# Hiroshiba/realtime-yukarin

Hardware: AMD Instinct MI355X
Metric: acoustic frames/s (stage1+stage2 fwd) @16kHz/5ms (higher is better)
Workload: dtype f32; 1 GPU; BASELINE config #3: stage-1 + stage-2 SR forward, buffer_time 0.5 s + 2x0.5 s convert_extra_time @16 kHz / 5 ms -> 300 real frames (384 padded) per window, 1 window(s) per GPU per step, SYN-64 random-init weights; model=SYN-64, frames=300, padded_frames=384, windows_per_gpu=1, lanes_per_gpu=2

## Files before the change

### realtime_yukarin_amd/csrc/ry_exec.cpp

```cpp
#include "ry_kernels.h"
#include "ry_plan.h"

static void fill_geom(RyConvGeom& g, const Layer& l, const LayerPlan& lp, int B, const float* s1, int C1, const float* s2, int C2) {
    memset(&g, 0, sizeof g);
    const TapTable t = make_taps(l);
    g.src1 = s1; g.src2 = s2; g.C1 = C1; g.C2 = C2; g.S1 = C1; g.S2 = C2;
    if (lp.path == PATH_IGEMM_BF16 && lp.x3) { g.C1 = 3 * C1; g.C2 = 3 * C2; g.S1 = 2 * C1; g.S2 = 2 * C2; }
    g.B = B; g.Hi = lp.Hi; g.Wi = lp.Wi; g.Ho = lp.Ho; g.Wo = lp.Wo;
    g.Hs = lp.Hi; g.Hos = lp.Ho;
    if (lp.crop_hi > 0) { g.Hi = lp.crop_hi; g.Ho = l.deconv ? 2 * lp.crop_hi : lp.crop_hi; }
    if (l.deconv) { g.Mh = g.Hi; g.Mw = lp.Wi; g.stride = 1; g.pad = 0; g.ostride = 2; }
    else { g.Mh = g.Ho; g.Mw = lp.Wo; g.stride = l.stride; g.pad = l.pad; g.ostride = 1; }
    g.nphases = t.nphases; g.ntaps = t.ntaps; g.N = l.cout; g.kw = l.deconv ? 2 : l.k; g.dil = l.deconv ? 1 : l.dil;
    const size_t esize = lp.path == PATH_IGEMM_BF16 ? 2 : 4;
    g.zoff1 = (unsigned)((size_t)B * lp.Hi * lp.Wi * g.S1 * esize); g.zoff2 = (unsigned)((size_t)B * lp.Hi * lp.Wi * g.S2 * esize);
    if (lp.crop_hi > 0 && lp.crop_lo > 0) {
        const size_t o1 = (size_t)lp.crop_lo * lp.Wi * g.S1 * esize, o2 = (size_t)lp.crop_lo * lp.Wi * g.S2 * esize;
        g.src1 = reinterpret_cast<const float*>(reinterpret_cast<const char*>(s1) + o1); g.zoff1 -= (unsigned)o1;
        if (s2) { g.src2 = reinterpret_cast<const float*>(reinterpret_cast<const char*>(s2) + o2); g.zoff2 -= (unsigned)o2; }
    }
    for (int ph = 0; ph < 4; ++ph) {
        g.pdy[ph] = (signed char)t.pdy[ph]; g.pdx[ph] = (signed char)t.pdx[ph];
        for (int tt = 0; tt < 16; ++tt) { g.tdy[ph][tt] = (signed char)t.dy[ph][tt]; g.tdx[ph][tt] = (signed char)t.dx[ph][tt]; }
    }
// ... 190 lines not shown
        while ((1 << p.tw_shift) < tw) ++p.tw_shift;
        p.th = th;
    }
    dim3 grid((unsigned)(((p.s.mtiles * p.s.ntiles * g.nphases * lp.splits + 7) / 8) * 8));
    RY_TRY(Lc.begin(tile_name(lp.tile, lp.kg, bf16, patch), l.name, lp.flops, lp.bytes, grid));
#define RY_IGEMM_LAUNCH(BM_, BN_, WM_, WN_, BF16_)                                                                                        \
    do {                                                                                                                                 \
        if (patch == 1 && lp.kg == 2) RY_LAUNCH((ry_igemm_ldsdma<BM_, BN_, WM_, WN_, 2, BF16_, 1>), grid, 512, Lc.stream, p);            \
        else if (patch == 1) RY_LAUNCH((ry_igemm_ldsdma<BM_, BN_, WM_, WN_, 1, BF16_, 1>), grid, 256, Lc.stream, p);                     \
        else if (patch == 2 && lp.kg == 2) RY_LAUNCH((ry_igemm_ldsdma<BM_, BN_, WM_, WN_, 2, BF16_, 2>), grid, 512, Lc.stream, p);       \
        else if (patch == 2) RY_LAUNCH((ry_igemm_ldsdma<BM_, BN_, WM_, WN_, 1, BF16_, 2>), grid, 256, Lc.stream, p);                     \
        else if (lp.kg == 2) RY_LAUNCH((ry_igemm_ldsdma<BM_, BN_, WM_, WN_, 2, BF16_, 0>), grid, 512, Lc.stream, p);                     \
        else RY_LAUNCH((ry_igemm_ldsdma<BM_, BN_, WM_, WN_, 1, BF16_, 0>), grid, 256, Lc.stream, p);                                     \
    } while (0)
#define RY_IGEMM_TILES(BF16_)                                                   \
    switch (lp.tile) {                                                          \
        case TILE_128x128: RY_IGEMM_LAUNCH(128, 128, 2, 2, BF16_); break;       \
        case TILE_96x128: RY_IGEMM_LAUNCH(96, 128, 1, 4, BF16_); break;         \
        case TILE_64x128: RY_IGEMM_LAUNCH(64, 128, 1, 4, BF16_); break;         \
        case TILE_128x64: RY_IGEMM_LAUNCH(128, 64, 4, 1, BF16_); break;         \
        default: RY_IGEMM_LAUNCH(32, 128, 1, 4, BF16_); break;                  \
    }
    if (bf16) RY_IGEMM_TILES(true) else RY_IGEMM_TILES(false)
#undef RY_IGEMM_TILES
#undef RY_IGEMM_LAUNCH
    RY_TRY(Lc.end());
    return launch_tail(Lc, l, lp, B, g.Ho, slope);
}

static int launch_conv2d(Launcher& Lc, const Layer& l, const LayerPlan& lp, int B, const float* s1, int C1, const float* s2, int C2, float slope) {
    if (lp.path == PATH_OS2D) return launch_c2d_os(Lc, l, lp, B, s1, C1, s2, C2, slope);
    if (lp.path == PATH_WINO) return launch_wino(Lc, l, lp, B, s1, C1, s2, C2, slope);
    if (lp.path == PATH_IGEMM || lp.path == PATH_IGEMM_BF16) return launch_igemm(Lc, l, lp, B, s1, C1, s2, C2, slope);
    if (lp.path == PATH_FIRST) {
        RySrFirstParams p;
        p.x = s1; p.w = l.wdir; p.scale = l.scale; p.shift = l.shift; p.out16 = lp.w16 ? lp.out16 : nullptr;
        p.out = (lp.w32 || !p.out16) ? lp.out : nullptr;
        p.x3 = lp.o16x3 ? 1 : 0;
        p.B = B; p.H = lp.Hi; p.W = lp.Wi; p.N = l.cout; p.act = l.act; p.slope = slope;
        const int quads = l.cout / 4;
        p.qshift = -1;
        for (int sh = 0; sh < 16; ++sh) if ((1 << sh) == quads) p.qshift = sh;
        const long long per_row = (long long)((lp.Wi + 3) / 4) * quads;
        dim3 grid((unsigned)((per_row + 255) / 256), (unsigned)lp.Hi, (unsigned)B);
        if (grid.y > 65535u || grid.z > 65535u) return fail(RY_EINVAL, "%s: %u rows x %u windows exceed the grid limit", l.name, grid.y, grid.z);
        RY_TRY(Lc.begin("ry_sr_first", l.name, lp.flops, lp.bytes, grid));
        RY_LAUNCH((ry_sr_first<4>), grid, 256, Lc.stream, p);
        RY_TRY(Lc.end());
    } else if (lp.path == PATH_LAST) {
        RySrLastParams p;
        p.src1 = s1; p.src2 = s2; p.C1 = C1; p.C2 = C2; p.w = l.wdir; p.scale = l.scale; p.shift = l.shift;
        p.out = lp.out; p.B = B; p.H = lp.Hi; p.W = lp.Wi;
        p.rows_valid = lp.last_rows; p.out_cols = lp.last_cols; p.do_exp = lp.last_exp;
        p.row0 = lp.last_row0; p.out_rows = lp.last_out_rows > 0 ? lp.last_out_rows : lp.last_rows;
        const long long total = (long long)B * p.rows_valid * lp.Wi;
        dim3 grid((unsigned)((total + 7) / 8));
        if (C1 + C2 == 128 && lp.Wi % 16 == 0) {
            const long long strips = (long long)B * p.rows_valid * (lp.Wi / 16);
            p.xcd_band = 1;
            const long long nb = (strips + 7) / 8;
            dim3 sg((unsigned)(((nb + 7) / 8) * 8));
            RY_TRY(Lc.begin("ry_sr_last<false>", l.name, lp.flops, lp.bytes, sg));
            RY_LAUNCH(ry_sr_last<false>, sg, 256, Lc.stream, p);
        } else {
            RY_TRY(Lc.begin("ry_sr_last_gather", l.name, lp.flops, lp.bytes, grid));
            RY_LAUNCH(ry_sr_last_gather, grid, 256, Lc.stream, p);
        }
// ... 76 lines not shown
            break;
        default:
            RY_OS_CASE_NU(RY_C1D_DECONV) RY_OS_CASE(RY_C1D_DECONV, 4, 4) RY_OS_CASE(RY_C1D_DECONV, 2, 8) RY_OS_CASE(RY_C1D_DECONV, 2, 4)
            return fail(RY_EINVAL, "%s: no ry_c1d_os instantiation for slice %dx%d", l.name, lp.os_cb, lp.os_tp);
            break;
    }
#undef RY_OS_CASE
#undef RY_OS_CASE_NU
#undef RY_OS_CASE_PM
    return Lc.end();
}

static RySrc1d src1d_of(const ry_net* net, const Plan& P, int idx) {
    RySrc1d s;
    memset(&s, 0, sizeof s);
    if (idx == -2) { s.C = 0; s.Craw = 1; s.splits = 1; return s; }
    if (idx == -1) {
        s.raw = P.mode == 1 ? P.x_in : P.cur_in; s.C = net->desc.in_ch; s.Craw = s.C; s.splits = 1; s.act = RY_ACT_NONE;
        return s;
    }
    const Layer& l = net->layers[idx];
    const LayerPlan& lp = P.lp[idx];
    s.raw = lp.raw; s.scale = l.scale; s.shift = l.shift; s.slab_stride = lp.slab_stride;
    s.C = l.act == RY_ACT_GLU ? l.cout / 2 : l.cout; s.Craw = l.cout; s.splits = lp.splits; s.act = l.act;
    return s;
}

static int enqueue_forward(ry_net* net, Plan& P, Launcher& Lc) {
    const ry_net_desc& d = net->desc;
    const int lo = 0, hi = 16;
    const int nd = d.ndim, B = P.B;
    const float slope = d.lrelu_slope;
    const bool padfuse_now = plan_padfuse_now(net, P);
    if (P.mode == 1 && !padfuse_now) {
        const int cols_in = nd == 1 ? d.in_ch : d.width + 1;
        const int cols_out = nd == 1 ? d.in_ch : d.width;
        RyPadRowsParams q;
        q.in = P.cur_in; q.minv = nullptr; q.out = P.x_in;
        q.rows_in = P.n_frames; q.cols_in = cols_in; q.rows_out = P.T; q.cols_out = cols_out; q.take_log = nd == 2;
        q.in_bstride = (long long)P.n_frames * cols_in; q.out_bstride = (long long)P.T * cols_out; q.minv_bstride = cols_in;
        dim3 pg((unsigned)((cols_in + 15) / 16), (unsigned)B);
        RY_TRY(Lc.begin("ry_pad_min_rows", "pad", 0, 4.0 * B * (P.n_frames * cols_in + P.T * cols_out), pg));
        if (P.n_frames > 128) RY_LAUNCH(ry_pad_min_rows<64>, pg, 1024, Lc.stream, q);
        else RY_LAUNCH(ry_pad_min_rows<16>, pg, 256, Lc.stream, q);
        RY_TRY(Lc.end());
    }
    const WindowRows rows = plan_window_rows(net, P);
    for (int i = lo; i < hi; ++i) {
        const Layer& l = net->layers[i];
        const LayerPlan& lp = P.lp[i];
        if (nd == 1 && P.s1_os) {
            const bool fused_pad = l.src_a < 0 && padfuse_now;
            const float* sa = l.src_a < 0 ? ((P.mode == 1 && !padfuse_now) ? P.x_in : P.cur_in) : P.lp[l.src_a].out;
            const float* sb = l.src_b < 0 ? nullptr : P.lp[l.src_b].out;
            const int keep = (i == 15 && P.mode == 1) ? P.n_frames : lp.Wo;
            RY_TRY(launch_c1d_os(Lc, l, lp, B, sa, l.cin_a, sb, l.cin_b, i == 15 ? P.cur_out : lp.out, keep, slope, fused_pad ? P.n_frames : 0));
        } else if (nd == 1) {
            RY_TRY(launch_conv1d(Lc, l, lp, B, src1d_of(net, P, l.src_a), src1d_of(net, P, l.src_b), slope));
        } else {
            const bool in16 = lp.path == PATH_IGEMM_BF16;
            const float* s1 = l.src_a < 0 ? (P.mode == 1 ? P.x_in : P.cur_in)
                                          : in16 ? reinterpret_cast<const float*>(P.lp[l.src_a].out16) : P.lp[l.src_a].out;
            const float* s2 = l.src_b < 0 ? nullptr : in16 ? reinterpret_cast<const float*>(P.lp[l.src_b].out16) : P.lp[l.src_b].out;
            LayerPlan lq = lp;
            if (i == 15 && (P.mode == 0 || lp.path == PATH_LAST)) lq.out = P.cur_out;
            if (i == 15 && P.mode == 1 && lp.path == PATH_LAST) {
                lq.last_rows = rows.k1 - rows.k0; lq.last_row0 = rows.k0; lq.last_out_rows = P.n_frames; lq.flops = lp.flops * (rows.k1 - rows.k0) / lp.Ho;
            }
            if (rows.hole_n[i] > 0) { lq.hole_lo = rows.hole_lo[i]; lq.hole_n = rows.hole_n[i]; lq.flops = lp.flops * (lp.Ho - rows.hole_n[i]) / lp.Ho; }
            if (rows.crop_hi[i] > 0) {
                lq.crop_hi = rows.crop_hi[i]; lq.crop_lo = rows.crop_lo[i]; lq.flops = lp.flops * rows.crop_hi[i] / lp.Hi; lq.bytes = lp.bytes * rows.crop_hi[i] / lp.Hi;
            }
            RY_TRY(launch_conv2d(Lc, l, lq, B, s1, l.cin_a, s2, l.cin_b, slope));
        }
    }
    if (nd == 1 && P.s1_os) {
    } else if (nd == 1) {
        RyMaterializeParams m;
        m.s = src1d_of(net, P, 15); m.L = P.T; m.keep = P.mode == 1 ? P.n_frames : P.T;
        m.npix = (long long)B * m.keep; m.slope = slope;
        m.out = P.cur_out;
        dim3 mg((unsigned)((m.npix * d.out_ch + 255) / 256));
        RY_TRY(Lc.begin("ry_materialize", "decoder/c7", 0, 4.0 * m.npix * d.out_ch * 2, mg));
        RY_LAUNCH(ry_materialize, mg, 256, Lc.stream, m);
        RY_TRY(Lc.end());
    } else if (P.mode == 1 && P.lp[15].path != PATH_LAST) {
        RySrPostParams q;
        q.y = P.lp[15].out; q.out = P.cur_out; q.rows = P.n_frames; q.cols_in = d.width; q.cols_out = d.width + 1;
        q.y_bstride = (long long)P.T * d.width; q.out_bstride = (long long)P.n_frames * (d.width + 1);
        dim3 pg((unsigned)(((long long)P.n_frames * (d.width + 1) + 255) / 256), (unsigned)B);
        RY_TRY(Lc.begin("ry_sr_post", "post", 0, 8.0 * B * P.n_frames * (d.width + 1), pg));
        RY_LAUNCH(ry_sr_post, pg, 256, Lc.stream, q);
        RY_TRY(Lc.end());
    }
    return RY_OK;
}

int autotune_plan(ry_net* net, Plan& P) {
    ry_ctx* ctx = net->ctx;
    const int B = P.B;
    const float slope = net->desc.lrelu_slope;
// ... 436 lines not shown
```

### realtime_yukarin_amd/csrc/ry_host.h

```cpp
#pragma once
#include "ry_dev.h"

#include "../../include/ry355.h"

#include <cmath>
#include <cstdarg>
#include <cstdio>
#include <cstdlib>
#include <chrono>
#include <cstring>
#include <map>
#include <memory>
#include <string>
#include <tuple>
#include <vector>

namespace rt {
#ifdef RY_HOST_EMU
typedef int err_t;
static const char* err_str(err_t) { return "emu"; }
static err_t set_device(int) { return 0; }
static err_t device_count(int* n) { *n = 1; return 0; }
static err_t stream_create(ry_stream_t* s) { *s = nullptr; return 0; }
static err_t stream_destroy(ry_stream_t) { return 0; }
// ... 125 lines not shown
    float* wigx3 = nullptr;
    int cin() const { return cin_a + cin_b; }
};

enum { PATH_IGEMM = 1, PATH_DIRECT = 2, PATH_FIRST = 3, PATH_LAST = 4, PATH_IGEMM_BF16 = 5,
       PATH_IGEMM_X3 = 6,
       PATH_OS2D = 7,
       PATH_WINO = 8 };
enum { TILE_128x128 = 1, TILE_64x128 = 3, TILE_32x128 = 4, TILE_128x64 = 5, TILE_96x128 = 6 };

struct LayerPlan {
    int Hi = 1, Wi = 1, Ho = 1, Wo = 1;
    int splits = 1;
    long long slab_stride = 0;
    float* raw = nullptr;
    int os_cb = 0, os_tp = 0, os_kt = 0;
    int path = 0, tile = 0;
    bool any_m_patch = false;
    int os2_mt4 = 0, os2_nt4 = 0, os2_waves = 0, os2_depth = 0;
    int wino_cfg = 0, wino_mbw = 0;
    const float* wwin = nullptr;
    int kg = 1;
    float* out = nullptr;
    unsigned short* out16 = nullptr;
    bool w32 = true, w16 = false;
    bool x3 = false;
    bool o16x3 = false;
    float* slabs = nullptr;
    int hole_lo = 0, hole_n = 0;
    int crop_hi = 0;
    int crop_lo = 0;
    int last_rows = 0, last_cols = 0, last_exp = 0;
    int last_row0 = 0, last_out_rows = 0;
    double flops = 0, bytes = 0;
    double flops_exec = 0;
};

inline void keep_rows(int n_frames, int disc_front, int disc_back, int* k0, int* k1) {
    *k0 = disc_front < n_frames ? disc_front : 0;
    *k1 = n_frames - disc_back > *k0 ? n_frames - disc_back : n_frames;
}

struct Plan {
    int B = 0, T = 0;
    int mode = 0;
    int n_frames = 0;
    int disc_front = 0, disc_back = 0;
    Arena arena;
    std::vector<LayerPlan> lp;
    float* user_in = nullptr;
    float* user_out = nullptr;
    float* x_in = nullptr;
    size_t user_in_floats = 0, user_out_floats = 0;
    bool s1_os = false;
    bool s1_padfuse = false;
    const float* cur_in = nullptr;
    float* cur_out = nullptr;
#ifndef RY_HOST_EMU
    struct GraphSlot { const float* in; float* out; hipGraphExec_t gexec; bool tried; long long graph_n, last_n; unsigned long long used; };
    std::vector<GraphSlot> gslots;
    unsigned long long gclock = 0;
    ~Plan() { for (GraphSlot& g : gslots) if (g.gexec) hipGraphExecDestroy(g.gexec); }
#endif
};

struct KernelRec {
    std::string name, layer;
    double flops, bytes, flops_exec;
    int grid[3];
};

struct ry_net {
    int dtype = 0;
    ry_ctx* ctx = nullptr;
    ry_stream_t stream = nullptr;
    rt::Event done;
    bool has_done = false;
    ry_net_desc desc;
    std::vector<Layer> layers;
    std::shared_ptr<Arena> weights = std::make_shared<Arena>();
    std::map<std::tuple<int, int, int, int>, std::unique_ptr<Plan>> plans;
    Plan* last_plan = nullptr;
    bool use_graph = true;
    std::vector<KernelRec>* rec = nullptr;
    std::vector<std::pair<rt::Event, rt::Event>>* rec_events = nullptr;
};

static int upload(Arena& a, ry_ctx* ctx, const std::vector<float>& h, float** d) {
// ... 35 lines not shown
```

### realtime_yukarin_amd/csrc/ry_kernels.h

```cpp
#pragma once
#include "ry_dev.h"


RY_DEV float ry_act(float v, int act, float slope) {
    if (act == RY_ACT_LRELU) return v >= 0.f ? v : v * slope;
    if (act == RY_ACT_RELU) return v > 0.f ? v : 0.f;
    return v;
}
RY_DEV float ry_sigmoid(float v) { return 1.f / (1.f + expf(-v)); }

RY_DEV int ry_fdiv(int x, int d, float inv_d) {
    int q = (int)((float)x * inv_d);
    const int r = x - q * d;
    q += (r >= d) ? 1 : 0;
    q -= (r < 0) ? 1 : 0;
    return q;
}

RY_DEV void ry_keep2(float& a, float& b) {
#ifndef RY_HOST_EMU
    asm volatile("" : "+v"(a), "+v"(b));
#endif
}
RY_DEV int ry_bitrev(int v, int bits) {
// ... 1068 lines not shown
    const int Ctot = g.C1 + g.C2;
    float acc = 0.f;
    for (int t = 0; t < g.ntaps; ++t) {
        const int iy = yb + g.tdy[phase][t], ix = xb + g.tdx[phase][t];
        if ((unsigned)iy >= (unsigned)g.Hi || (unsigned)ix >= (unsigned)g.Wi) continue;
        const size_t pix = (size_t)(b * g.Hs + iy) * g.Wi + ix;
        const float* w = p.wd + ((size_t)(phase * g.ntaps + t) * Ctot) * g.N + n;
        const float* s1 = g.src1 + pix * g.C1;
        for (int c = 0; c < g.C1; ++c) acc = fmaf(s1[c], w[(size_t)c * g.N], acc);
        if (g.C2 > 0) {
            const float* s2 = g.src2 + pix * g.C2;
            const float* w2 = w + (size_t)g.C1 * g.N;
            for (int c = 0; c < g.C2; ++c) acc = fmaf(s2[c], w2[(size_t)c * g.N], acc);
        }
    }
    const size_t ob = (size_t)(b * g.Hos + ry * g.ostride + g.pdy[phase]) * g.Wo + rx * g.ostride + g.pdx[phase];
    p.out[ob * g.N + n] = ry_act(fmaf(acc, p.scale[n], p.shift[n]), p.act, p.slope);
}

struct RySrFirstParams {
    const float* x;
    const float* w;
    const float* scale;
    const float* shift;
    float* out;
    unsigned short* out16;
    int x3;
    int B, H, W, N;
    int act;
    float slope;
    int qshift;
};

template <int PX>
RY_KERNEL(256) void ry_sr_first(RySrFirstParams p) {
    const int quads = p.N >> 2;
    const int gpr = (p.W + PX - 1) / PX;
    const int idx = (int)blockIdx.x * 256 + (int)threadIdx.x;
    const int gx = p.qshift >= 0 ? idx >> p.qshift : idx / quads;
    const int cq = idx - gx * quads;
    if (gx >= gpr) return;
    const int y = (int)blockIdx.y, b = (int)blockIdx.z;
    const int x0 = gx * PX;
    f32x4 wr[9];
#pragma unroll
    for (int t = 0; t < 9; ++t) wr[t] = ry_ld4(p.w + (size_t)t * p.N + cq * 4);
    const f32x4 sc = ry_ld4(p.scale + cq * 4), sh = ry_ld4(p.shift + cq * 4);
    float xv[3][PX + 2];
#pragma unroll
    for (int dy = 0; dy < 3; ++dy) {
        const int iy = y + dy - 1;
#pragma unroll
        for (int j = 0; j < PX + 2; ++j) {
            const int ix = x0 + j - 1;
            xv[dy][j] = ((unsigned)iy < (unsigned)p.H && (unsigned)ix < (unsigned)p.W) ? p.x[((size_t)b * p.H + iy) * p.W + ix] : 0.f;
        }
    }
#pragma unroll
    for (int j = 0; j < PX; ++j) {
        if (x0 + j >= p.W) break;
        f32x4 acc = {0.f, 0.f, 0.f, 0.f};
#pragma unroll
        for (int t = 0; t < 9; ++t) {
            const float xs_ = xv[t / 3][j + t % 3];
#pragma unroll
            for (int u = 0; u < 4; ++u) acc[u] = fmaf(xs_, wr[t][u], acc[u]);
        }
        f32x4 o;
#pragma unroll
        for (int u = 0; u < 4; ++u) o[u] = ry_act(fmaf(acc[u], sc[u], sh[u]), p.act, p.slope);
        const size_t oi = (((size_t)b * p.H + y) * p.W + x0 + j) * p.N + cq * 4;
        if (p.out) ry_st4(p.out + oi, o);
        if (p.out16) {
            if (p.x3) ry_st4_bf16_x3(p.out16, ((size_t)b * p.H + y) * p.W + x0 + j, p.N, cq * 4, o);
            else ry_st4_bf16(p.out16 + oi, o);
        }
    }
}

struct RySrLastParams {
    const float* src1;
    const float* src2;
    int C1, C2;
    const float* w;
    const float* scale;
    const float* shift;
    float* out;
    int B, H, W;
    int rows_valid;
    int row0;
    int out_rows;
    int out_cols;
    int do_exp;
    int xcd_band;
};

RY_KERNEL(256) void ry_sr_last_gather(RySrLastParams p) {
    const int l = (int)threadIdx.x & 31;
    const long long pix = (long long)blockIdx.x * 8 + (threadIdx.x >> 5);
    const long long total = (long long)p.B * p.rows_valid * p.W;
    const bool live = pix < total;
    const long long pp = live ? pix : 0;
    const int x = (int)(pp % p.W);
    const int y = (int)((pp / p.W) % p.rows_valid) + p.row0;
    const int b = (int)(pp / ((long long)p.W * p.rows_valid));
    const int Ctot = p.C1 + p.C2;
    float acc = 0.f;
    if (live) {
        for (int t = 0; t < 9; ++t) {
// ... 630 lines not shown
```

### realtime_yukarin_amd/csrc/ry_plan.cpp

```cpp
#include "ry_plan.h"

static const int ENC_CH[8] = {1, 2, 4, 8, 8, 8, 8, 8};
static const int DEC_IN[7] = {8, 16, 16, 16, 16, 8, 4};
static const int DEC_OUT[7] = {8, 8, 8, 8, 4, 2, 1};

std::vector<Layer> build_topology(const ry_net_desc& d) {
    std::vector<Layer> L(16);
    const int B = d.base, e = d.extensive_layers;
    const int end_k = e > 0 ? 3 : 1;
    const int g = (d.glu && d.ndim == 1) ? 2 : 1;
    const int blk_act_e = g == 2 ? RY_ACT_GLU : RY_ACT_LRELU, blk_act_d = g == 2 ? RY_ACT_GLU : RY_ACT_RELU;
    auto nm = [](Layer& l, const char* p, int i) { snprintf(l.name, sizeof l.name, "%s/c%d", p, i); };
    {
        Layer& l = L[0]; nm(l, "encoder", 0);
        l.k = end_k; l.stride = 1; l.pad = end_k / 2; l.cin_a = d.in_ch; l.cout = B; l.src_a = -1; l.act = RY_ACT_LRELU;
    }
    for (int i = 1; i < 8; ++i) {
        Layer& l = L[i]; nm(l, "encoder", i);
        const bool down = i < e;
        l.k = down ? 4 : 1; l.stride = down ? 2 : 1; l.pad = down ? 1 : 0;
        l.cin_a = ENC_CH[i - 1] * B; l.cout = ENC_CH[i] * B * g; l.src_a = i - 1; l.bn = true; l.act = blk_act_e;
    }
    for (int j = 0; j < 7; ++j) {
        Layer& l = L[8 + j]; nm(l, "decoder", j);
// ... 228 lines not shown
        relayout_direct(l, W, w);
        RY_TRY(upload(arena, ctx, w, &l.wdir));
    }
    return RY_OK;
}

static int g_poison = 0;
int poison_fill(ry_ctx* ctx, float* p, size_t nfloats) {
    if (!g_poison || !p || !nfloats) return RY_OK;
    RT_TRY(rt::dmemset(p, 0xFF, nfloats * sizeof(float), ctx->stream));
    RT_TRY(rt::stream_sync(ctx->stream));
    return RY_OK;
}
int alloc_ztail(ry_ctx* ctx, Arena& arena, float** p, size_t nfloats) {
    RY_TRY(arena.alloc(p, nfloats + ZTAIL));
    if (g_poison) RT_TRY(rt::dmemset(*p, 0xFF, nfloats * sizeof(float), ctx->stream));
    RT_TRY(rt::dmemset(*p + nfloats, 0, ZTAIL * sizeof(float), ctx->stream));
    RT_TRY(rt::stream_sync(ctx->stream));
    return RY_OK;
}

void tile_dims(int tile, int* bm, int* bn) {
    switch (tile) {
        case TILE_128x128: *bm = 128; *bn = 128; break;
        case TILE_64x128: *bm = 64; *bn = 128; break;
        case TILE_128x64: *bm = 128; *bn = 64; break;
        case TILE_96x128: *bm = 96; *bn = 128; break;
        default: *bm = 32; *bn = 128; break;
    }
}


static int g_s2_hole = 1;
static int g_s2_crop = 2;
static LayerForce g_force[16];
bool layer_plan_fixed(int i) { return g_force[i].fixed(); }
int g_x3_min_m = 128;
int g_autotune = 0;
int g_autotune_reps = 3, g_autotune_max = 0;
int g_autotune_pick = -1;
const char* tile_name(int tile, int kg, bool bf16, int patch) {
    {
        static std::map<int, std::string> names;
        const int key = ((tile * 4 + kg) * 2 + (bf16 ? 1 : 0)) * 4 + patch;
        auto it = names.find(key);
        if (it == names.end()) {
            int bm, bn; tile_dims(tile, &bm, &bn);
            const int wmv = (tile == TILE_128x128) ? 2 : (tile == TILE_128x64 ? 4 : 1), wnv = 4 / wmv;
            char buf[96];
            snprintf(buf, sizeof buf, "ry_igemm_ldsdma<%d,%d,%d,%d,%d,%s,%d>", bm, bn, wmv, wnv, kg == 2 ? 2 : 1, bf16 ? "true" : "false", patch);
            it = names.emplace(key, buf).first;
        }
        return it->second.c_str();
    }
}

static thread_local double g_plan_peak = 157.3e6;
static thread_local int g_plan_ck = 32;
static const double g_x3_peak = 2.0e9, g_x3_kg2 = 1.15;
static thread_local double g_plan_kg2 = 1.0;

int tile_occ(int tile, int kg) {
    int bm, bn; tile_dims(tile, &bm, &bn);
    const int occ = (160 * 1024) / (kg * (bm + bn) * 32 * 4 * 2 + bm * 16);
    const int cap = 4 / kg;
    return occ > cap ? cap : occ;
// ... 224 lines not shown

static int ensure_wwin(ry_net* net, int i, const float** out) {
    auto& lazy = net->weights->lazy;
    auto it = lazy.find(i);
    if (it == lazy.end()) {
        float* d = nullptr;
        RY_TRY(upload_wwin(net->ctx, *net->weights, net->layers[i], &d));
        it = lazy.emplace(i, d).first;
    }
    *out = it->second;
    return RY_OK;
}

bool plan_tile_rows(const LayerPlan& lp, int Mh, int Mw, int* th, int* tw_out) {
    if (lp.path == PATH_WINO) {
        int tw; wino_tile_hw(lp.wino_cfg, lp.wino_mbw, th, &tw);
        if (tw_out) *tw_out = tw;
        return Mh % *th == 0 && Mw % tw == 0;
    }
    int bm, bn; tile_dims(lp.tile, &bm, &bn);
    for (int tw = 16; tw >= 4; tw >>= 1)
        if (bm % tw == 0 && Mw % tw == 0 && Mh % (bm / tw) == 0) { *th = bm / tw; if (tw_out) *tw_out = tw; return true; }
    return false;
}

bool plan_hole_ok(const Layer& l, const LayerPlan& lp, int lo, int n) {
    const bool igemm = lp.path == PATH_IGEMM || lp.path == PATH_IGEMM_BF16;
    if ((!igemm && lp.path != PATH_WINO) || (igemm && lp.splits != 1) || l.deconv || lp.crop_hi > 0 || (lp.Wo * l.cout) % 8) return false;
    int th = 1, tw = 0;
    if (!plan_tile_rows(lp, lp.Ho, lp.Wo, &th, &tw) || (igemm && tw != 16)) return false;
    return n > 0 && lo >= 1 && lo % th == 0 && n % th == 0 && lo + n <= lp.Ho;
}

WindowRows plan_window_rows(const ry_net* net, const Plan& P) {
    const int nd = net->desc.ndim, B = P.B;
    WindowRows w;
    w.k1 = P.n_frames;
    if (nd == 2 && P.mode == 1 && P.lp[15].path == PATH_LAST) {
        keep_rows(P.n_frames, P.disc_front, P.disc_back, &w.k0, &w.k1);
    }
    if (nd == 2 && P.mode == 1 && g_s2_crop && P.lp[15].path == PATH_LAST && net->layers[15].src_a == 14) {
        int need0 = w.k0 > 0 ? w.k0 - 1 : 0, need1 = w.k1 + 1;
        for (int i = 14; i >= 8; --i) {
            const Layer& l = net->layers[i];
            const LayerPlan& lp = P.lp[i];
            if (need1 > lp.Ho) need1 = lp.Ho;
            if (need0 <= 0 && need1 >= lp.Ho) break;
            if (lp.path != PATH_IGEMM && lp.path != PATH_IGEMM_BF16 && lp.path != PATH_WINO) break;
            if (l.src_a != i - 1) break;
            int r0, r1;
            if (l.deconv) { r0 = need0 > 0 ? (need0 - 1) / 2 : 0; r1 = need1 / 2 + 1; }
            else if (l.k == 1 && l.stride == 1) { r0 = need0; r1 = need1; }
            else break;
            const int Mw = l.deconv ? lp.Wi : lp.Wo, Mh = l.deconv ? lp.Hi : lp.Ho;
            int th = 1;
            if (plan_tile_rows(lp, Mh, Mw, &th)) { r0 = r0 / th * th; r1 = (r1 + th - 1) / th * th; }
            if (r1 > lp.Hi) r1 = lp.Hi;
            if (r0 <= 0 && r1 >= lp.Hi) break;
            int bm = 256, bn = 64;
            if (lp.path == PATH_WINO) { if (lp.wino_cfg == 2) bm = 512; } else tile_dims(lp.tile, &bm, &bn);
            const long wgs = (long)(((long)B * Mh * Mw + bm - 1) / bm) * (l.cout / bn) * (l.deconv ? 4 : 1) * lp.splits;
            if (g_s2_crop >= 2 || wgs > 256) { w.crop_lo[i] = r0; w.crop_hi[i] = r1 - r0; need0 = r0; need1 = r1; }
            else { need0 = 0; need1 = lp.Hi; }
        }
    }
    if (nd == 2 && P.mode == 1 && g_s2_hole && P.n_frames < P.T - 2) {
// ... 111 lines not shown
    }
    if (nd == 1) {
        P.s1_os = true;
        for (int i = 0; i < 16; ++i) if (!c1d_os_capable(net->layers[i]) || !net->layers[i].w1os) P.s1_os = false;
        P.s1_padfuse = P.s1_os && P.mode == 1 && c1d_mode(net->layers[0]) == RY_C1D_S1 && net->layers[0].cin() <= 64;
    }
    for (int i = 0; i < 16; ++i) {
        const Layer& l = net->layers[i];
        LayerPlan& lp = P.lp[i];
        const size_t out_elems = (size_t)B * lp.Ho * lp.Wo * l.cout;
        if (nd == 1 && P.s1_os) {
            plan_s1_os(l, lp, B);
            if (i < 15) {
                RY_TRY(P.arena.alloc(&lp.out, out_elems));
                RY_TRY(poison_fill(net->ctx, lp.out, out_elems));
            }
        } else if (nd == 1) {
            const int mode = c1d_mode(l);
            lp.splits = choose_splits_1d(l, B, mode == RY_C1D_DECONV ? lp.Wi : lp.Wo, mode);
            lp.slab_stride = (long long)out_elems;
            RY_TRY(P.arena.alloc(&lp.raw, out_elems * lp.splits));
            RY_TRY(poison_fill(net->ctx, lp.raw, out_elems * lp.splits));
        } else {
            RY_TRY(alloc_ztail(net->ctx, P.arena, &lp.out, out_elems));
            bool src16 = l.src_a >= 0;
            for (int src : {l.src_a, l.src_b}) {
                const int sp = src >= 0 ? P.lp[src].path : 0;
                if (src >= 0 && sp != PATH_FIRST && sp != PATH_IGEMM && sp != PATH_IGEMM_BF16 && sp != PATH_OS2D) src16 = false;
            }
            RY_TRY(plan_s2_layer(net->ctx, P.arena, l, lp, B, net->dtype, g_force[i], src16, i == 15, P.mode));
            if (lp.path == PATH_WINO) RY_TRY(ensure_wwin(net, i, &lp.wwin));
        }
    }
    if (nd == 2 && net->dtype != 0) {
        const bool x3 = net->dtype == 2;
        std::vector<char> need32(16, 0), need16(16, 0);
        need32[15] = 1;
        for (int i = 0; i < 16; ++i)
            for (int src : {net->layers[i].src_a, net->layers[i].src_b})
                if (src >= 0) (P.lp[i].path == PATH_IGEMM_BF16 ? need16 : need32)[src] = 1;
        for (int i = 0; i < 16; ++i) {
            LayerPlan& lp = P.lp[i];
            lp.w32 = need32[i] || lp.path == PATH_DIRECT || lp.path == PATH_LAST; lp.w16 = need16[i];
            lp.o16x3 = x3;
            if (lp.w16) {
                float* q = nullptr;
                RY_TRY(alloc_ztail(net->ctx, P.arena, &q, ((size_t)B * lp.Ho * lp.Wo * net->layers[i].cout * (x3 ? 2 : 1) + 1) / 2));
                lp.out16 = reinterpret_cast<unsigned short*>(q);
            }
        }
    }
    const int cin_user = nd == 1 ? d.in_ch : (P.mode == 1 ? d.width + 1 : d.width);
    const int cout_user = nd == 1 ? d.out_ch : (P.mode == 1 ? d.width + 1 : d.width);
    const int rows_user = P.T;
    P.user_in_floats = (size_t)B * rows_user * cin_user;
    P.user_out_floats = (size_t)B * rows_user * cout_user;
    RY_TRY(P.arena.alloc(&P.user_in, P.user_in_floats));
    RY_TRY(P.arena.alloc(&P.user_out, P.user_out_floats));
    if (P.mode == 1) {
        RY_TRY(P.arena.alloc(&P.x_in, (size_t)B * P.T * (nd == 1 ? d.in_ch : d.width)));
        RY_TRY(poison_fill(net->ctx, P.x_in, (size_t)B * P.T * (nd == 1 ? d.in_ch : d.width)));
    } else {
        P.x_in = nullptr;
    }
    return RY_OK;
}
// ... 17 lines not shown
    if (const char* e = getenv("RY_WINOGRAD")) g_wino = atoi(e);
    if (const char* e = getenv("RY_WINO_MINM")) g_wino_min_m = atoi(e);
    RY_TRY(parse_force("RY_WINO", "layer:cfg[:mbw[:splits]][,...]", [](LayerForce& f, const int* v) {
        if (v[0] < 0 || v[0] > 2 || v[1] < 0 || v[2] < 0) return false;
        f.wino_set = true; f.wino[0] = v[0]; f.wino[1] = v[1]; f.wino[2] = v[2];
        return true;
    }));
    g_poison = 0;
    if (const char* e = getenv("RY_POISON")) g_poison = atoi(e);
    RY_TRY(parse_force("RY_OS2", "layer:mt4[:nt4[:waves[:depth]]][,...]", [](LayerForce& f, const int* v) {
        if (v[0] < 0 || v[1] < 0 || v[2] < 0 || v[3] < 0) return false;
        f.os2_set = true; f.os2[0] = v[0]; f.os2[1] = v[1]; f.os2[2] = v[2]; f.os2[3] = v[3];
        return true;
    }));
    return parse_force("RY_PLAN", "layer:tile:splits:kgroups[,...]", [](LayerForce& f, const int* v) {
        if (v[0] < 0 || v[0] > TILE_96x128 || v[0] == 2 || v[1] < 0 || v[2] < 0 || v[2] > 2) return false;
        f.tile = v[0]; f.splits = v[1]; f.kg = v[2];
        return true;
    });
}

int read_env_switches() {
    g_autotune = 0; g_autotune_reps = 3; g_autotune_max = 0; g_autotune_pick = -1;
    if (const char* e = getenv("RY_AUTOTUNE")) {
        int on = 0, reps = 3, mx = 0, pick = -1;
        if (sscanf(e, "%d:%d:%d:%d", &on, &reps, &mx, &pick) < 1) return fail(RY_EINVAL, "RY_AUTOTUNE: expected 1[:reps[:max[:pick]]]");
        g_autotune = on; g_autotune_reps = reps > 0 ? reps : 1; g_autotune_max = mx; g_autotune_pick = pick;
    }
    g_x3_min_m = 128; g_s2_crop = 2;
    if (const char* e = getenv("RY_X3_MINM")) g_x3_min_m = atoi(e);
    if (const char* e = getenv("RY_S2_CROP")) g_s2_crop = atoi(e);
    g_s2_hole = 1;
    if (const char* e = getenv("RY_S2_HOLE")) g_s2_hole = atoi(e);
    return read_plan_env();
}

unsigned short host_f2bf(float f) {
    unsigned u; memcpy(&u, &f, 4);
    if ((u & 0x7fffffffu) > 0x7f800000u) return (unsigned short)((u >> 16) | 0x40);
    u += 0x7fffu + ((u >> 16) & 1u);
    return (unsigned short)(u >> 16);
}

float host_bf2f(unsigned short h) { const unsigned u = (unsigned)h << 16; float f; memcpy(&f, &u, 4); return f; }

static void build_wig16(const Layer& l, const std::vector<float>& w32, std::vector<unsigned short>& out) {
    const TapTable t = make_taps(l);
    const int C = l.cin(), N = l.cout;
    const size_t outer = (size_t)t.nphases * (N / 64) * t.ntaps;
    out.assign(outer * (size_t)C * 64, 0);
    for (size_t o = 0; o < outer; ++o)
        for (int c = 0; c < C; ++c)
            for (int nl = 0; nl < 64; ++nl)
                out[(o * (C / 64) + c / 64) * 4096 + wig16_inblock(nl, c % 64)] = host_f2bf(w32[(o * (C / 32) + c / 32) * 2048 + wig_inblock(nl, c % 32)]);
}

static void build_wigx3(const Layer& l, const std::vector<float>& w32, std::vector<unsigned short>& out) {
    const TapTable t = make_taps(l);
    const int C = l.cin(), N = l.cout, K3 = 3 * C;
    const size_t outer = (size_t)t.nphases * (N / 64) * t.ntaps;
    out.assign(outer * (size_t)K3 * 64, 0);
    for (size_t o = 0; o < outer; ++o)
        for (int kk = 0; kk < K3; ++kk) {
            int seg, c;
            if (kk < 3 * l.cin_a) { seg = kk / l.cin_a; c = kk % l.cin_a; }
            else { const int k2 = kk - 3 * l.cin_a; seg = k2 / l.cin_b; c = l.cin_a + k2 % l.cin_b; }
// ... 25 lines not shown
```

### realtime_yukarin_amd/csrc/ry_plan.h

```cpp
#pragma once
#include "ry_dev.h"
#include "ry_host.h"

struct TapTable {
    int nphases = 1, ntaps = 1;
    int dy[4][16], dx[4][16], ky[4][16], kx[4][16], pdy[4], pdx[4];
};

static const size_t ZTAIL = 2048;

#define RY_OS2_CONFIGS(X)                                                                                              \
    X(1, 1, 4, 4) X(1, 1, 8, 4) X(1, 1, 8, 2) X(1, 1, 16, 2) X(2, 1, 4, 4) X(2, 1, 8, 4) X(2, 1, 8, 2) X(2, 1, 16, 2)     \
    X(3, 1, 4, 4) X(3, 1, 8, 4) X(3, 1, 8, 2) X(3, 1, 16, 2) X(4, 1, 4, 4) X(4, 1, 8, 4) X(4, 1, 8, 2) X(4, 1, 16, 2)     \
    X(6, 1, 4, 4) X(6, 1, 8, 2)                                                             \
    X(1, 2, 4, 4) X(1, 2, 8, 4) X(1, 2, 8, 2) X(1, 2, 16, 2) X(2, 2, 4, 4) X(2, 2, 8, 4) X(2, 2, 8, 2) X(2, 2, 16, 2)     \
    X(3, 2, 4, 4) X(3, 2, 8, 4) X(3, 2, 8, 2) X(3, 2, 16, 2) X(4, 2, 4, 4) X(4, 2, 8, 4) X(4, 2, 8, 2) X(4, 2, 16, 2)     \
    X(6, 2, 4, 4) X(6, 2, 8, 2)                                                                             \
    X(1, 4, 4, 4) X(1, 4, 8, 4) X(1, 4, 8, 2) X(1, 4, 16, 2) X(2, 4, 4, 4) X(2, 4, 8, 4) X(2, 4, 8, 2) X(2, 4, 16, 2)     \
    X(3, 4, 4, 4) X(3, 4, 8, 4) X(3, 4, 8, 2) X(4, 4, 4, 4) X(4, 4, 8, 2) X(6, 4, 4, 2)

static constexpr bool os2_xl_ok(int mt4, int waves, int depth) { return depth == 2 && mt4 * waves <= 32; }

struct LayerForce {
    int tile = 0, splits = 0, kg = 0;
// ... 14 lines not shown
int check_desc(const ry_net_desc* d);
TapTable make_taps(const Layer& l);
bool wino_eligible(const Layer& l, int ndim);
int prepare_layer(ry_ctx* ctx, Arena& arena, Layer& l, int ndim, float eps, const float* W, const float* b, const float* bn, bool want_os2 = false);
int prepare_bf16(ry_ctx* ctx, Arena& arena, Layer& l, int dtype);
int upload_wwin(ry_ctx* ctx, Arena& arena, const Layer& l, float** out);
int alloc_ztail(ry_ctx* ctx, Arena& arena, float** p, size_t nfloats);
int poison_fill(ry_ctx* ctx, float* p, size_t nfloats);
void tile_dims(int tile, int* bm, int* bn);
extern int g_x3_min_m;
extern int g_autotune;
extern int g_autotune_reps, g_autotune_max;
extern int g_autotune_pick;
bool layer_plan_fixed(int i);
const char* tile_name(int tile, int kg, bool bf16, int patch);
int tile_occ(int tile, int kg);
double est_time(long blocks, int bm, int bn, int s, int occ, int kg, int M, int N, int nk);
void choose_igemm(const Layer& l, int M, int nphases, int nk, int* tile, int* splits, int* kg, int bf16 = 0 );
bool choose_os2(int M, int N, int nphases, int U, int* mt4, int* nt4, int* waves, int* depth, double* cost_out = nullptr);
bool wino_cfg_dims(int cfg, int* wm, int* wn, int* nsl);
void wino_tile_hw(int cfg, int mbw, int* th, int* tw);
const char* wino_name(int cfg, int mode);
bool choose_wino(int Mh, int Mw, int N, int nphases, int npatches, int B, int* cfg, int* mbw, int* splits);
int c1d_mode(const Layer& l);
int c1d_tile_len(int mode);
int choose_splits_1d(const Layer& l, int B, int rows, int mode);
bool c1d_os_capable(const Layer& l);
void plan_s1_os(const Layer& l, LayerPlan& lp, int B);
bool plan_tile_rows(const LayerPlan& lp, int Mh, int Mw, int* th, int* tw_out = nullptr);
bool plan_hole_ok(const Layer& l, const LayerPlan& lp, int lo, int n);
int plan_s2_layer(ry_ctx* ctx, Arena& arena, const Layer& l, LayerPlan& lp, int B, int dtype, const LayerForce& f, bool src16, bool out_layer, int mode);
WindowRows plan_window_rows(const ry_net* net, const Plan& P);
inline bool plan_padfuse_now(const ry_net* net, const Plan& P) { return net->desc.ndim == 1 && P.s1_padfuse && P.n_frames <= 2048; }
int build_plan(ry_net* net, Plan& P);
int autotune_plan(ry_net* net, Plan& P);
int get_plan(ry_net* net, int B, int T, int mode, int n_frames, Plan** out);
int run_plan(ry_net* net, Plan& P, const float* x, float* y, int on_device);
int read_plan_env();
int read_env_switches();
unsigned short host_f2bf(float f);
float host_bf2f(unsigned short h);
int profile_plan(ry_net* net, Plan* P, int reps, ry_kernel_stat* stats, int max_stats, int* n_stats);
```

Measured before the change: 348,500 frames/s.

## Fuse stage-2 pad/min/log preprocessing into the first SR conv kernel

For stage-2 the separate pad-rows kernel (log, pad with column minimum) is skipped and its work is folded into a new first-layer kernel. Real rows apply the log on the fly while the conv runs and write x_in. Dedicated tail blocks compute the column minimum and produce the constant padded rows. Since padded rows are all identical, interior outputs are computed once per pixel and broadcast across rows. This removes one launch and a round trip through memory. In exchange the kernel is more complex, the tail blocks do a serial min-reduction, and work is uneven across blocks.

```diff
diff --git a/realtime_yukarin_amd/csrc/ry_exec.cpp b/realtime_yukarin_amd/csrc/ry_exec.cpp
--- a/realtime_yukarin_amd/csrc/ry_exec.cpp
+++ b/realtime_yukarin_amd/csrc/ry_exec.cpp
@@ -246,7 +246,29 @@
     if (lp.path == PATH_OS2D) return launch_c2d_os(Lc, l, lp, B, s1, C1, s2, C2, slope);
     if (lp.path == PATH_WINO) return launch_wino(Lc, l, lp, B, s1, C1, s2, C2, slope);
     if (lp.path == PATH_IGEMM || lp.path == PATH_IGEMM_BF16) return launch_igemm(Lc, l, lp, B, s1, C1, s2, C2, slope);
-    if (lp.path == PATH_FIRST) {
+    if (lp.path == PATH_FIRST && lp.head_raw) {
+        RySrFirstPadParams p;
+        memset(&p, 0, sizeof p);
+        p.raw = lp.head_raw; p.x_in = lp.head_xin; p.n = lp.head_n; p.cols_in = lp.head_cols;
+        p.w = l.wdir; p.scale = l.scale; p.shift = l.shift; p.out16 = lp.w16 ? lp.out16 : nullptr;
+        p.out = (lp.w32 || !p.out16) ? lp.out : nullptr;
+        p.x3 = lp.o16x3 ? 1 : 0;
+        p.B = B; p.H = lp.Hi; p.W = lp.Wi; p.N = l.cout; p.act = l.act; p.slope = slope;
+        const int quads = l.cout / 4;
+        p.qshift = -1;
+        for (int sh = 0; sh < 16; ++sh) if ((1 << sh) == quads) p.qshift = sh;
+        if (p.qshift < 0 || lp.Wi % 4 || p.n < 1 || p.n >= lp.Hi || p.cols_in < lp.Wi || !p.x_in)
+            return fail(RY_ESTATE, "%s: not a shape for the fused head (width %d, %d channels, %d of %d rows)", l.name, lp.Wi, l.cout, p.n, lp.Hi);
+        const long long per_row = (long long)(lp.Wi / 4) * quads;
+        p.gx = (int)((per_row + 255) / 256); p.tail_blocks = (lp.Wi + 7) / 8;
+        const long long blocks = (long long)p.tail_blocks + (long long)p.gx * (p.n - 1);
+        if (blocks >= (1ll << 31) || (unsigned)B > 65535u) return fail(RY_EINVAL, "%s: %lld workgroups x %d windows exceed the grid limit", l.name, blocks, B);
+        dim3 grid((unsigned)blocks, 1, (unsigned)B);
+        const int rows_run = p.n - 1 + (lp.Hi - p.n >= 3 ? 4 : lp.Hi - p.n + 1);
+        RY_TRY(Lc.begin("ry_sr_first_pad", l.name, lp.flops * rows_run / lp.Hi, lp.bytes + 4.0 * B * p.n * p.cols_in, grid));
+        RY_LAUNCH((ry_sr_first_pad<4>), grid, 256, Lc.stream, p);
+        RY_TRY(Lc.end());
+    } else if (lp.path == PATH_FIRST) {
         RySrFirstParams p;
         p.x = s1; p.w = l.wdir; p.scale = l.scale; p.shift = l.shift; p.out16 = lp.w16 ? lp.out16 : nullptr;
         p.out = (lp.w32 || !p.out16) ? lp.out : nullptr;
@@ -389,7 +411,8 @@
     const int nd = d.ndim, B = P.B;
     const float slope = d.lrelu_slope;
     const bool padfuse_now = plan_padfuse_now(net, P);
-    if (P.mode == 1 && !padfuse_now) {
+    const bool headfuse_now = plan_headfuse_now(net, P);
+    if (P.mode == 1 && !padfuse_now && !headfuse_now) {
         const int cols_in = nd == 1 ? d.in_ch : d.width + 1;
         const int cols_out = nd == 1 ? d.in_ch : d.width;
         RyPadRowsParams q;
@@ -424,6 +447,7 @@
             if (i == 15 && P.mode == 1 && lp.path == PATH_LAST) {
                 lq.last_rows = rows.k1 - rows.k0; lq.last_row0 = rows.k0; lq.last_out_rows = P.n_frames; lq.flops = lp.flops * (rows.k1 - rows.k0) / lp.Ho;
             }
+            if (i == 0 && headfuse_now) { lq.head_raw = P.cur_in; lq.head_xin = P.x_in; lq.head_n = P.n_frames; lq.head_cols = d.width + 1; }
             if (rows.hole_n[i] > 0) { lq.hole_lo = rows.hole_lo[i]; lq.hole_n = rows.hole_n[i]; lq.flops = lp.flops * (lp.Ho - rows.hole_n[i]) / lp.Ho; }
             if (rows.crop_hi[i] > 0) {
                 lq.crop_hi = rows.crop_hi[i]; lq.crop_lo = rows.crop_lo[i]; lq.flops = lp.flops * rows.crop_hi[i] / lp.Hi; lq.bytes = lp.bytes * rows.crop_hi[i] / lp.Hi;
diff --git a/realtime_yukarin_amd/csrc/ry_host.h b/realtime_yukarin_amd/csrc/ry_host.h
--- a/realtime_yukarin_amd/csrc/ry_host.h
+++ b/realtime_yukarin_amd/csrc/ry_host.h
@@ -181,6 +181,9 @@
     int crop_lo = 0;
     int last_rows = 0, last_cols = 0, last_exp = 0;
     int last_row0 = 0, last_out_rows = 0;
+    const float* head_raw = nullptr;
+    float* head_xin = nullptr;
+    int head_n = 0, head_cols = 0;
     double flops = 0, bytes = 0;
     double flops_exec = 0;
 };
@@ -203,6 +206,7 @@
     size_t user_in_floats = 0, user_out_floats = 0;
     bool s1_os = false;
     bool s1_padfuse = false;
+    bool s2_headfuse = false;
     const float* cur_in = nullptr;
     float* cur_out = nullptr;
 #ifndef RY_HOST_EMU
diff --git a/realtime_yukarin_amd/csrc/ry_kernels.h b/realtime_yukarin_amd/csrc/ry_kernels.h
--- a/realtime_yukarin_amd/csrc/ry_kernels.h
+++ b/realtime_yukarin_amd/csrc/ry_kernels.h
@@ -1124,6 +1124,28 @@
     int qshift;
 };
 
+RY_DEV f32x4 ry_sr_first_px(const f32x4* wr, const float* x9, f32x4 sc, f32x4 sh, int act, float slope) {
+    f32x4 acc = {0.f, 0.f, 0.f, 0.f};
+#pragma unroll
+    for (int t = 0; t < 9; ++t) {
+        const float xs_ = x9[t];
+#pragma unroll
+        for (int u = 0; u < 4; ++u) acc[u] = fmaf(xs_, wr[t][u], acc[u]);
+    }
+    f32x4 o;
+#pragma unroll
+    for (int u = 0; u < 4; ++u) o[u] = ry_act(fmaf(acc[u], sc[u], sh[u]), act, slope);
+    return o;
+}
+RY_DEV void ry_sr_first_st(float* out, unsigned short* out16, int x3, size_t pix, int N, int c0, f32x4 o) {
+    const size_t oi = pix * (size_t)N + c0;
+    if (out) ry_st4(out + oi, o);
+    if (out16) {
+        if (x3) ry_st4_bf16_x3(out16, pix, N, c0, o);
+        else ry_st4_bf16(out16 + oi, o);
+    }
+}
+
 template <int PX>
 RY_KERNEL(256) void ry_sr_first(RySrFirstParams p) {
     const int quads = p.N >> 2;
@@ -1151,22 +1173,139 @@
 #pragma unroll
     for (int j = 0; j < PX; ++j) {
         if (x0 + j >= p.W) break;
-        f32x4 acc = {0.f, 0.f, 0.f, 0.f};
-#pragma unroll
-        for (int t = 0; t < 9; ++t) {
-            const float xs_ = xv[t / 3][j + t % 3];
-#pragma unroll
-            for (int u = 0; u < 4; ++u) acc[u] = fmaf(xs_, wr[t][u], acc[u]);
-        }
-        f32x4 o;
-#pragma unroll
-        for (int u = 0; u < 4; ++u) o[u] = ry_act(fmaf(acc[u], sc[u], sh[u]), p.act, p.slope);
-        const size_t oi = (((size_t)b * p.H + y) * p.W + x0 + j) * p.N + cq * 4;
-        if (p.out) ry_st4(p.out + oi, o);
-        if (p.out16) {
-            if (p.x3) ry_st4_bf16_x3(p.out16, ((size_t)b * p.H + y) * p.W + x0 + j, p.N, cq * 4, o);
-            else ry_st4_bf16(p.out16 + oi, o);
-        }
+        float x9[9];
+#pragma unroll
+        for (int t = 0; t < 9; ++t) x9[t] = xv[t / 3][j + t % 3];
+        const f32x4 o = ry_sr_first_px(wr, x9, sc, sh, p.act, p.slope);
+        ry_sr_first_st(p.out, p.out16, p.x3, ((size_t)b * p.H + y) * p.W + x0 + j, p.N, cq * 4, o);
+    }
+}
+
+struct RySrFirstPadParams {
+    const float* raw;
+    float* x_in;
+    const float* w;
+    const float* scale;
+    const float* shift;
+    float* out;
+    unsigned short* out16;
+    int x3;
+    int B, H, W, N;
+    int n, cols_in;
+    int act;
+    float slope;
+    int qshift;
+    int gx;
+    int tail_blocks;
+};
+
+template <int PX>
+RY_KERNEL(256) void ry_sr_first_pad(RySrFirstPadParams p) {
+    constexpr int TB = 8;
+    __shared__ float red[256];
+    __shared__ float rowA[16], rowB[16], rowF[16];
+    const int tid = (int)threadIdx.x, b = (int)blockIdx.z;
+    const int quads = p.N >> 2;
+    const float* raw = p.raw + (size_t)b * (size_t)p.n * p.cols_in;
+    float* xin = p.x_in + (size_t)b * (size_t)p.H * p.W;
+    if ((int)blockIdx.x < p.tail_blocks) {
+        const int c0 = (int)blockIdx.x * TB;
+        {
+            const int cl = tid & 15, grp = tid >> 4;
+            const int c = c0 - 1 + cl;
+            const bool live = cl < TB + 2 && c >= 0 && c < p.W;
+            float m = INFINITY;
+            for (int r0 = grp; r0 < p.n; r0 += 8 * 16) {
+                float v[8];
+#pragma unroll
+                for (int u = 0; u < 8; ++u) { const int r = r0 + 16 * u; v[u] = (live && r < p.n) ? raw[(size_t)r * p.cols_in + c] : INFINITY; }
+#pragma unroll
+                for (int u = 0; u < 8; ++u) m = fminf(m, v[u]);
+            }
+            red[tid] = m;
+            if (grp == 1) rowB[cl] = live ? logf(raw[(size_t)(p.n - 1) * p.cols_in + c]) : 0.f;
+            if (grp == 2) rowA[cl] = (live && p.n >= 2) ? logf(raw[(size_t)(p.n - 2) * p.cols_in + c]) : 0.f;
+            __syncthreads();
+            if (grp == 0) {
+                float mm = red[cl];
+#pragma unroll
+                for (int g = 1; g < 16; ++g) mm = fminf(mm, red[g * 16 + cl]);
+                rowF[cl] = live ? logf(mm) : 0.f;
+            }
+            __syncthreads();
+        }
+        for (int e = tid; e < (p.H - p.n + 1) * TB; e += 256) {
+            const int r = p.n - 1 + (e >> 3), j = e & (TB - 1);
+            if (c0 + j < p.W) xin[(size_t)r * p.W + c0 + j] = r == p.n - 1 ? rowB[j + 1] : rowF[j + 1];
+        }
+        auto xrow = [&](int iy, int cl) -> float {
+            return (iy < 0 || iy >= p.H) ? 0.f : iy >= p.n ? rowF[cl] : iy == p.n - 1 ? rowB[cl] : rowA[cl];
+        };
+        const int ish = p.qshift + 3, items = 1 << ish;
+        for (int it = tid; it < 3 * items; it += 256) {
+            const int slot = it >> ish, px = (it >> p.qshift) & (TB - 1), cq = it & (quads - 1);
+            const int y = slot == 0 ? p.n - 1 : slot == 1 ? p.n : p.H - 1;
+            if ((slot == 2 && y <= p.n) || c0 + px >= p.W) continue;
+            f32x4 wr[9];
+#pragma unroll
+            for (int t = 0; t < 9; ++t) wr[t] = ry_ld4(p.w + (size_t)t * p.N + cq * 4);
+            const f32x4 sc = ry_ld4(p.scale + cq * 4), sh = ry_ld4(p.shift + cq * 4);
+            float x9[9];
+#pragma unroll
+            for (int t = 0; t < 9; ++t) x9[t] = xrow(y + t / 3 - 1, px + t % 3);
+            const f32x4 o = ry_sr_first_px(wr, x9, sc, sh, p.act, p.slope);
+            ry_sr_first_st(p.out, p.out16, p.x3, ((size_t)b * p.H + y) * p.W + c0 + px, p.N, cq * 4, o);
+        }
+        if (p.H - 2 >= p.n + 1) {
+            const int rstep = items >= 256 ? 1 : 256 >> ish, rl = items >= 256 ? 0 : tid >> ish;
+            for (int it = items >= 256 ? tid : (tid & (items - 1)); it < items; it += 256) {
+                const int px = it >> p.qshift, cq = it & (quads - 1);
+                if (c0 + px >= p.W) continue;
+                f32x4 wr[9];
+#pragma unroll
+                for (int t = 0; t < 9; ++t) wr[t] = ry_ld4(p.w + (size_t)t * p.N + cq * 4);
+                const f32x4 sc = ry_ld4(p.scale + cq * 4), sh = ry_ld4(p.shift + cq * 4);
+                float x9[9];
+#pragma unroll
+                for (int t = 0; t < 9; ++t) x9[t] = rowF[px + t % 3];
+                const f32x4 o = ry_sr_first_px(wr, x9, sc, sh, p.act, p.slope);
+                for (int y = p.n + 1 + rl; y <= p.H - 2; y += rstep)
+                    ry_sr_first_st(p.out, p.out16, p.x3, ((size_t)b * p.H + y) * p.W + c0 + px, p.N, cq * 4, o);
+            }
+        }
+        return;
+    }
+    const int bi = (int)blockIdx.x - p.tail_blocks;
+    const int y = bi / p.gx;
+    const int idx = (bi - y * p.gx) * 256 + tid;
+    const int gx = idx >> p.qshift, cq = idx & (quads - 1);
+    if (gx >= p.W / PX) return;
+    const int x0 = gx * PX;
+    f32x4 wr[9];
+#pragma unroll
+    for (int t = 0; t < 9; ++t) wr[t] = ry_ld4(p.w + (size_t)t * p.N + cq * 4);
+    const f32x4 sc = ry_ld4(p.scale + cq * 4), sh = ry_ld4(p.shift + cq * 4);
+    float xv[3][PX + 2];
+#pragma unroll
+    for (int dy = 0; dy < 3; ++dy) {
+        const int iy = y + dy - 1;
+#pragma unroll
+        for (int j = 0; j < PX + 2; ++j) {
+            const int ix = x0 + j - 1;
+            xv[dy][j] = (iy >= 0 && (unsigned)ix < (unsigned)p.W) ? logf(raw[(size_t)iy * p.cols_in + ix]) : 0.f;
+        }
+    }
+    if (cq == 0) {
+#pragma unroll
+        for (int j = 0; j < PX; ++j) xin[(size_t)y * p.W + x0 + j] = xv[1][j + 1];
+    }
+#pragma unroll
+    for (int j = 0; j < PX; ++j) {
+        float x9[9];
+#pragma unroll
+        for (int t = 0; t < 9; ++t) x9[t] = xv[t / 3][j + t % 3];
+        const f32x4 o = ry_sr_first_px(wr, x9, sc, sh, p.act, p.slope);
+        ry_sr_first_st(p.out, p.out16, p.x3, ((size_t)b * p.H + y) * p.W + x0 + j, p.N, cq * 4, o);
     }
 }
 
diff --git a/realtime_yukarin_amd/csrc/ry_plan.cpp b/realtime_yukarin_amd/csrc/ry_plan.cpp
--- a/realtime_yukarin_amd/csrc/ry_plan.cpp
+++ b/realtime_yukarin_amd/csrc/ry_plan.cpp
@@ -284,6 +284,7 @@
 
 
 static int g_s2_hole = 1;
+static int g_s2_fuse_head = 1;
 static int g_s2_crop = 2;
 static LayerForce g_force[16];
 bool layer_plan_fixed(int i) { return g_force[i].fixed(); }
@@ -574,6 +575,10 @@
     return n > 0 && lo >= 1 && lo % th == 0 && n % th == 0 && lo + n <= lp.Ho;
 }
 
+bool plan_headfuse_now(const ry_net* net, const Plan& P) {
+    return net->desc.ndim == 2 && P.mode == 1 && P.s2_headfuse && g_s2_fuse_head && P.n_frames >= 1 && P.n_frames < P.T;
+}
+
 WindowRows plan_window_rows(const ry_net* net, const Plan& P) {
     const int nd = net->desc.ndim, B = P.B;
     WindowRows w;
@@ -751,6 +756,11 @@
             if (lp.path == PATH_WINO) RY_TRY(ensure_wwin(net, i, &lp.wwin));
         }
     }
+    if (nd == 2) {
+        const Layer& l0 = net->layers[0];
+        const int quads = l0.cout / 4;
+        P.s2_headfuse = P.mode == 1 && P.lp[0].path == PATH_FIRST && l0.src_a < 0 && d.width % 4 == 0 && l0.cout % 4 == 0 && quads > 0 && (quads & (quads - 1)) == 0;
+    }
     if (nd == 2 && net->dtype != 0) {
         const bool x3 = net->dtype == 2;
         std::vector<char> need32(16, 0), need16(16, 0);
@@ -834,6 +844,8 @@
     if (const char* e = getenv("RY_S2_CROP")) g_s2_crop = atoi(e);
     g_s2_hole = 1;
     if (const char* e = getenv("RY_S2_HOLE")) g_s2_hole = atoi(e);
+    g_s2_fuse_head = 1;
+    if (const char* e = getenv("RY_S2_FUSE_HEAD")) g_s2_fuse_head = atoi(e);
     return read_plan_env();
 }
 
diff --git a/realtime_yukarin_amd/csrc/ry_plan.h b/realtime_yukarin_amd/csrc/ry_plan.h
--- a/realtime_yukarin_amd/csrc/ry_plan.h
+++ b/realtime_yukarin_amd/csrc/ry_plan.h
@@ -70,6 +70,7 @@
 int plan_s2_layer(ry_ctx* ctx, Arena& arena, const Layer& l, LayerPlan& lp, int B, int dtype, const LayerForce& f, bool src16, bool out_layer, int mode);
 WindowRows plan_window_rows(const ry_net* net, const Plan& P);
 inline bool plan_padfuse_now(const ry_net* net, const Plan& P) { return net->desc.ndim == 1 && P.s1_padfuse && P.n_frames <= 2048; }
+bool plan_headfuse_now(const ry_net* net, const Plan& P);
 int build_plan(ry_net* net, Plan& P);
 int autotune_plan(ry_net* net, Plan& P);
 int get_plan(ry_net* net, int B, int T, int mode, int n_frames, Plan** out);
```

Result: no change. 347,200 frames/s (-0.4%).
